# mantasu/face-crop-plus

Measured on AMD Instinct MI355X. Metric: faces/sec end-to-end (detect+align+crop), higher is better.
Workload: dtype f16x3; 1 GPU; RetinaFace detect + 5-pt align/crop, batch=32/GPU synthetic 1024x1024 RGB, strategy=largest, det_threshold=0.6, output 256x256, detector on 2 HIP streams x 16 images; global_batch=32, image_size=1024, parallelism=dp1

## Files before the change

face-crop-plus_amd/csrc/fcp_stem_pool.hip:

```cpp
#include "fcp_conv_common.h"

using namespace fcp_conv;

namespace {

typedef _Float16 f16x2 __attribute__((ext_vector_type(2)));

constexpr int PH = 5;
constexpr int SH = 2 * PH + 1;
constexpr int IH = 2 * SH + 5;
constexpr int SPITCH = 68;
constexpr int KSTEPS = 11;

struct StemGeo {
  static constexpr int PW = 16;
  static constexpr int SW = 2 * PW + 1;
  static constexpr int NSTEM = SH * SW;
  static constexpr int NTILES = (NSTEM + 31) / 32;
  static constexpr int IWB = (2 * SW + 5) * 3;
  static constexpr int IPITCH = 6 * SW + 18;
  static constexpr int IN_ELEMS = (IH + 1) * IPITCH;
  static constexpr int NT = 32 * PW;
  static constexpr int NGRP = NT / 128;
  static constexpr int TPR = NT / 28;
  static constexpr int NLOAD = (IWB + TPR - 1) / TPR;
  static constexpr int C1ROWS = (PH * PW + 31) / 32 * 32;
  static constexpr int C1_BYTES = C1ROWS * 2 * 128;
  static constexpr int WGS = 1;
  static_assert(TPR % 3 == 0 && IH * TPR <= NT && IPITCH % 2 == 0 && NTILES % NGRP == 0, "stem patch geometry");
};

struct StemParams {
  const uint8_t* img;
  const float* imgf;
  const uint32_t* wfrag;
  const float* bias;
  const float* wscale;
  float* out;
  int n, h, w, hs, ws, hp, wp, out_ld, out_fmt;
  int tiles_y, tiles_x, npatches;
  int mean[3];
  const char* w1;
  const float* ws1;
  const float* b1;
  float* t1;
  int t1_ld;
};

constexpr int CPITCH = 68;
__device__ __forceinline__ int swz1(int row) { return ((row >> 1) & 7) ^ ((row & 1) << 2); }

__device__ __forceinline__ void lds_barrier() {
  asm volatile("s_waitcnt lgkmcnt(0)" ::: "memory");
  __builtin_amdgcn_s_barrier();
  asm volatile("" ::: "memory");
}

template <bool HAS_C1, bool F32IN = false>
__global__ void __launch_bounds__(StemGeo::NT, StemGeo::WGS) stem_pool_kernel(const StemParams p) {
  static_assert(!(HAS_C1 && F32IN), "the fp32-input stem has no conv1 tail");
  using G = StemGeo;
  constexpr int PW = G::PW, SW = G::SW, NSTEM = G::NSTEM, NTILES = G::NTILES, IWB = G::IWB, IPITCH = G::IPITCH;
  constexpr int IN_ELEMS = G::IN_ELEMS, NT = G::NT, NGRP = G::NGRP, TPR = G::TPR, NLOAD = G::NLOAD, C1ROWS = G::C1ROWS;
  constexpr int KPG = NTILES / NGRP;
  extern __shared__ __attribute__((aligned(16))) float smem[];
  __shared__ __attribute__((aligned(16))) _Float16 inh[IN_ELEMS];
  __shared__ __attribute__((aligned(16))) _Float16 inl[F32IN ? IN_ELEMS : 8];
  float* stage = smem;
  char* c1in = reinterpret_cast<char*>(smem + NSTEM * SPITCH);

  const int tid = threadIdx.x;
  const int lane = tid & 63;
  const int wave = __builtin_amdgcn_readfirstlane(tid >> 6);
  const int half = lane >> 5;

  const int ct = wave & 1, grp = wave >> 1;
  f16x8 wh[KSTEPS], wl[KSTEPS];
#pragma unroll
  for (int q = 0; q < KSTEPS; ++q) {
    const u32x4_t* src = reinterpret_cast<const u32x4_t*>(p.wfrag) + ((ct * KSTEPS + q) * 2) * 64 + lane;
    wh[q] = __builtin_bit_cast(f16x8, src[0]);
    wl[q] = __builtin_bit_cast(f16x8, src[64]);
  }

  const int pc2 = 2 * (tid & 31), pcol = tid >> 5;
  const float ws2a = p.wscale[pc2], ws2b = p.wscale[pc2 + 1], bias2a = p.bias[pc2], bias2b = p.bias[pc2 + 1];
  float ws1a = 0.f, ws1b = 0.f, b1a = 0.f, b1b = 0.f;
  if constexpr (HAS_C1) { ws1a = p.ws1[pc2]; ws1b = p.ws1[pc2 + 1]; b1a = p.b1[pc2]; b1b = p.b1[pc2 + 1]; }
  const int c1rt = wave >> 1, c1ct = wave & 1;

  const int frow = tid / TPR, fc0 = tid - frow * TPR;
  const int fx0 = fc0 / 3, fch = fc0 - fx0 * 3;
  const int fmean = fch == 0 ? p.mean[0] : (fch == 1 ? p.mean[1] : p.mean[2]);
  _Float16* const fdst = inh + min(frow, IH - 1) * IPITCH + fc0;
  uint8_t pre[F32IN ? 1 : NLOAD];
  float pref[F32IN ? NLOAD : 1];
  unsigned pre_ok = 0u;
  auto fetch = [&](int patch) {
    const int pxi = patch % p.tiles_x;
    const int pyi = (patch / p.tiles_x) % p.tiles_y;
    const int ni = patch / (p.tiles_x * p.tiles_y);
    const int iy0 = 4 * pyi * PH - 5, ix0 = 4 * pxi * PW - 5;
    const int y = iy0 + frow;
    const bool rowok = (unsigned)y < (unsigned)p.h && frow < IH;
    const int yc = min(max(y, 0), p.h - 1);
    const uint8_t* base = p.img + ((long)ni * p.h + yc) * p.w * 3 + fch;
    const float* basef = p.imgf + ((long)ni * p.h + yc) * p.w * 4 + fch;
    pre_ok = 0u;
#pragma unroll
    for (int j = 0; j < NLOAD; ++j) {
      const int x = ix0 + fx0 + (TPR / 3) * j;
      pre_ok |= (rowok && (unsigned)x < (unsigned)p.w) ? (1u << j) : 0u;
      if constexpr (F32IN) pref[j] = basef[(unsigned)(min(max(x, 0), p.w - 1) * 4)];
      else pre[j] = base[(unsigned)(min(max(x, 0), p.w - 1) * 3)];
    }
  };
  _Float16* const fdstl = inl + (F32IN ? min(frow, IH - 1) * IPITCH + fc0 : 0);
  auto commit = [&]() {
    if (frow < IH) {
#pragma unroll
      for (int j = 0; j < NLOAD; ++j) {
        if (fc0 + TPR * j < IWB) {
          if constexpr (F32IN) {
            const float v = ((pre_ok >> j) & 1u) ? pref[j] : 0.f;
            const unsigned hu = __builtin_bit_cast(unsigned, __builtin_amdgcn_cvt_pkrtz(v, 0.f));
            const unsigned lu = __builtin_bit_cast(unsigned, __builtin_amdgcn_cvt_pkrtz(fcp_mix_diff<0>(v, hu), 0.f));
            fdst[TPR * j] = __builtin_bit_cast(_Float16, (unsigned short)(hu & 0xFFFFu));
            fdstl[TPR * j] = __builtin_bit_cast(_Float16, (unsigned short)(lu & 0xFFFFu));
          } else {
            fdst[TPR * j] = (_Float16)(float)(((pre_ok >> j) & 1u) ? (int)pre[j] - fmean : 0);
          }
        }
      }
    }
  };

  for (int i = tid; i < IN_ELEMS / 2; i += NT) {
    reinterpret_cast<uint32_t*>(inh)[i] = 0u;
    if constexpr (F32IN) reinterpret_cast<uint32_t*>(inl)[i] = 0u;
  }
  __syncthreads();

  int abase_t[KPG];
#pragma unroll
  for (int k = 0; k < KPG; ++k) {
    int pix = (grp + NGRP * k) * 32 + (lane & 31);
    pix = pix < NSTEM ? pix : NSTEM - 1;
    const int si = pix / SW, sj = pix - si * SW;
    abase_t[k] = (2 * si) * IPITCH + 6 * sj;
  }

  int patch = blockIdx.x;
  if (patch < p.npatches) fetch(patch);
  for (; patch < p.npatches; patch += gridDim.x) {
    commit();
    lds_barrier();
    const int next = patch + gridDim.x;
    if (next < p.npatches) fetch(next);

    const int pxi = patch % p.tiles_x;
    const int pyi = (patch / p.tiles_x) % p.tiles_y;
    const int ni = patch / (p.tiles_x * p.tiles_y);
    const int py0 = pyi * PH, px0 = pxi * PW;
    const int sy0 = 2 * py0 - 1, sx0 = 2 * px0 - 1;
    const bool interior = sy0 >= 0 && sy0 + SH <= p.hs && sx0 >= 0 && sx0 + SW <= p.ws;

#pragma unroll
    for (int k = 0; k < KPG; ++k) {
      const int t = grp + NGRP * k;
      const int abase = abase_t[k];
      f32x16 acc;
#pragma unroll
      for (int e = 0; e < 16; ++e) acc[e] = 0.f;
      auto afrag_of = [&](const _Float16* plane, int q) {
        const int ch = 2 * q + half;
        const int kh = ch / 3, part = ch - kh * 3;
        const uint32_t* wp = reinterpret_cast<const uint32_t*>(plane + abase + kh * IPITCH + 8 * part);
        const u32x4_t raw = {wp[0], wp[1], wp[2], wp[3]};
        return __builtin_bit_cast(f16x8, raw);
      };
      auto afrag = [&](int q) { return afrag_of(inh, q); };
      f16x8 a = afrag(0), al = a;
      if constexpr (F32IN) al = afrag_of(inl, 0);
#pragma unroll
      for (int q = 0; q < KSTEPS; ++q) {
        f16x8 an = a, aln = al;
        if (q + 1 < KSTEPS) {
          an = afrag(q + 1);
          if constexpr (F32IN) aln = afrag_of(inl, q + 1);
        }
        __builtin_amdgcn_sched_barrier(0);
        if constexpr (F32IN) {
          acc = __builtin_amdgcn_mfma_f32_32x32x16_f16(wh[q], al, acc, 0, 0, 0);
          acc = __builtin_amdgcn_mfma_f32_32x32x16_f16(wl[q], a, acc, 0, 0, 0);
          acc = __builtin_amdgcn_mfma_f32_32x32x16_f16(wh[q], a, acc, 0, 0, 0);
        } else {
          acc = __builtin_amdgcn_mfma_f32_32x32x16_f16(wl[q], a, acc, 0, 0, 0);
          acc = __builtin_amdgcn_mfma_f32_32x32x16_f16(wh[q], a, acc, 0, 0, 0);
        }
        a = an; al = aln;
      }
      {
        const int row = t * 32 + (lane & 31);
        bool in = true;
        if (!interior) {
          const int si = row / SW, sj = row - si * SW;
          in = (unsigned)(sy0 + si) < (unsigned)p.hs && (unsigned)(sx0 + sj) < (unsigned)p.ws;
        }
        if (row < NSTEM) {
          float* dst = stage + row * SPITCH + ct * 32 + 4 * half;
#pragma unroll
          for (int g = 0; g < 4; ++g)
            *reinterpret_cast<f32x4*>(dst + 8 * g) = in ? f32x4{acc[4 * g], acc[4 * g + 1], acc[4 * g + 2], acc[4 * g + 3]}
                                                        : f32x4{-INFINITY, -INFINITY, -INFINITY, -INFINITY};
        }
      }
    }
    lds_barrier();

    f16x8 c1w[8];
    if constexpr (HAS_C1) {
      if (c1rt < C1ROWS / 32) {
        const char* wrow = p.w1 + (size_t)(c1ct * 32 + (lane & 31)) * 256;
#pragma unroll
        for (int sl = 0; sl < 2; ++sl)
#pragma unroll
          for (int sh = 0; sh < 2; ++sh) {
            c1w[(sl * 2 + sh) * 2] = *reinterpret_cast<const f16x8*>(wrow + sl * 128 + (2 * sh + half) * 16);
            c1w[(sl * 2 + sh) * 2 + 1] = *reinterpret_cast<const f16x8*>(wrow + sl * 128 + (4 + 2 * sh + half) * 16);
          }
      }
    }
    {
      typedef float f32x2 __attribute__((ext_vector_type(2)));
      const float* sp = stage + (2 * pcol) * SPITCH + pc2;
      f32x2 rm[SH];
#pragma unroll
      for (int si = 0; si < SH; ++si) {
        const f32x2 a = *reinterpret_cast<const f32x2*>(sp + (si * SW) * SPITCH);
        const f32x2 b = *reinterpret_cast<const f32x2*>(sp + (si * SW + 1) * SPITCH);
        const f32x2 c = *reinterpret_cast<const f32x2*>(sp + (si * SW + 2) * SPITCH);
        rm[si][0] = fmaxf(fmaxf(a[0], b[0]), c[0]);
        rm[si][1] = fmaxf(fmaxf(a[1], b[1]), c[1]);
      }
      const int ox = px0 + pcol;
#pragma unroll
      for (int py = 0; py < PH; ++py) {
        const int oy = py0 + py;
        if (oy >= p.hp || ox >= p.wp) continue;
        float v0 = fmaxf(fmaxf(rm[2 * py][0], rm[2 * py + 1][0]), rm[2 * py + 2][0]) * ws2a + bias2a;
        float v1 = fmaxf(fmaxf(rm[2 * py][1], rm[2 * py + 1][1]), rm[2 * py + 2][1]) * ws2b + bias2b;
        v0 = v0 > 0.f ? v0 : 0.f;
        v1 = v1 > 0.f ? v1 : 0.f;
        const long pixel = ((long)ni * p.hp + oy) * p.wp + ox;
        if (p.out_fmt == 1) {
          unsigned hu, lu;
          split2(v0, v1, hu, lu);
          char* ob = reinterpret_cast<char*>(p.out) + pixel * p.out_ld * 4 + split_chan_off(pc2);
          *reinterpret_cast<unsigned*>(ob) = hu;
          *reinterpret_cast<unsigned*>(ob + 64) = lu;
          if constexpr (HAS_C1) {
            const int pp = py * PW + pcol;
            const int q = (pc2 & 31) >> 3, sw = swz1(pp);
            char* trow = c1in + pp * 256 + (pc2 >> 5) * 128 + (pc2 & 7) * 2;
            *reinterpret_cast<unsigned*>(trow + ((q ^ sw) << 4)) = hu;
            *reinterpret_cast<unsigned*>(trow + (((4 + q) ^ sw) << 4)) = lu;
          }
        } else {
          *reinterpret_cast<f32x2*>(p.out + pixel * p.out_ld + pc2) = f32x2{v0, v1};
        }
      }
    }
    if constexpr (HAS_C1) {
      lds_barrier();
      if (c1rt < C1ROWS / 32) {
        f32x16 acc;
#pragma unroll
        for (int e = 0; e < 16; ++e) acc[e] = 0.f;
        const int row = c1rt * 32 + (lane & 31), sw = swz1(row);
        const char* arow = c1in + row * 256;
#pragma unroll
        for (int sl = 0; sl < 2; ++sl)
#pragma unroll
          for (int sh = 0; sh < 2; ++sh) {
            const f16x8 bh = c1w[(sl * 2 + sh) * 2], bl = c1w[(sl * 2 + sh) * 2 + 1];
            const f16x8 ah = *reinterpret_cast<const f16x8*>(arow + sl * 128 + (((2 * sh + half) ^ sw) << 4));
            const f16x8 al = *reinterpret_cast<const f16x8*>(arow + sl * 128 + (((4 + 2 * sh + half) ^ sw) << 4));
            acc = __builtin_amdgcn_mfma_f32_32x32x16_f16(bh, al, acc, 0, 0, 0);
            acc = __builtin_amdgcn_mfma_f32_32x32x16_f16(bl, ah, acc, 0, 0, 0);
            acc = __builtin_amdgcn_mfma_f32_32x32x16_f16(bh, ah, acc, 0, 0, 0);
          }
        float* dst = stage + row * CPITCH + c1ct * 32 + 4 * half;
#pragma unroll
        for (int g = 0; g < 4; ++g)
          *reinterpret_cast<f32x4*>(dst + 8 * g) = f32x4{acc[4 * g], acc[4 * g + 1], acc[4 * g + 2], acc[4 * g + 3]};
      }
      lds_barrier();
      {
        typedef float f32x2 __attribute__((ext_vector_type(2)));
        const int ox = px0 + pcol;
        f32x2 cv[PH];
#pragma unroll
        for (int py = 0; py < PH; ++py) cv[py] = *reinterpret_cast<const f32x2*>(stage + (py * PW + pcol) * CPITCH + pc2);
#pragma unroll
        for (int py = 0; py < PH; ++py) {
          const int oy = py0 + py;
          if (oy >= p.hp || ox >= p.wp) continue;
          const float x0 = conv_value_relu(cv[py][0], ws1a, b1a), x1 = conv_value_relu(cv[py][1], ws1b, b1b);
          unsigned hu, lu;
          split2(x0, x1, hu, lu);
          const long pixel = ((long)ni * p.hp + oy) * p.wp + ox;
          char* ob = reinterpret_cast<char*>(p.t1) + pixel * p.t1_ld * 4 + split_chan_off(pc2);
          *reinterpret_cast<unsigned*>(ob) = hu;
          *reinterpret_cast<unsigned*>(ob + 64) = lu;
        }
      }
    }
    lds_barrier();
  }
}

}

extern "C" int fcp_stem7x7s2_relu_pool_conv1_u8(const uint8_t* images, int n, int h, int w, const int32_t* mean_rgb,
                                                const void* wfrag, const float* bias, const float* wscale, float* out,
                                                int out_ld, int out_fmt, const void* w1, const float* ws1, const float* b1,
                                                float* t1, int t1_ld, fcp_stream_t stream) {
  FCP_REQUIRE(images && wfrag && bias && wscale && out && mean_rgb, "stem: null pointer");
  const bool has_c1 = w1 != nullptr;
  if (has_c1) {
    FCP_REQUIRE(ws1 && b1 && t1, "stem + conv1: conv1 needs its scales, bias and output");
    FCP_REQUIRE(out_fmt == 1, "stem + conv1: the pooled map must be written in split32 (its bytes are conv1's operand)");
    FCP_REQUIRE(t1_ld >= 64 && t1_ld % 32 == 0 && ((uintptr_t)t1 & 127) == 0 && ((uintptr_t)w1 & 15) == 0,
                "stem + conv1: misaligned conv1 filter / output view");
  }
  FCP_REQUIRE(n > 0 && h >= 1 && w >= 1 && (long)h * w * 3 < (1L << 31), "stem: bad image size");
  FCP_REQUIRE((unsigned)out_fmt <= 1u, "stem: out_fmt must be 0 (fp32) or 1 (split32)");
  FCP_REQUIRE(out_ld >= 64 && out_ld % (out_fmt ? 32 : 4) == 0 && ((uintptr_t)out & (out_fmt ? 127 : 15)) == 0,
              "stem: misaligned output view");
  FCP_REQUIRE(((uintptr_t)wfrag & 15) == 0, "stem: filter fragments must be 16-byte aligned");
  for (int c = 0; c < 3; ++c) FCP_REQUIRE(mean_rgb[c] >= 0 && mean_rgb[c] <= 255, "stem: means must be integers in 0..255");
  StemParams p = {};
  p.img = images; p.wfrag = static_cast<const uint32_t*>(wfrag); p.bias = bias; p.wscale = wscale; p.out = out;
  p.n = n; p.h = h; p.w = w;
  p.hs = (h + 6 - 7) / 2 + 1; p.ws = (w + 6 - 7) / 2 + 1;
  p.hp = (p.hs + 2 - 3) / 2 + 1; p.wp = (p.ws + 2 - 3) / 2 + 1;
  p.out_ld = out_ld; p.out_fmt = out_fmt;
  p.tiles_y = fcp_cdiv(p.hp, PH); p.tiles_x = fcp_cdiv(p.wp, StemGeo::PW);
  const long np = (long)n * p.tiles_y * p.tiles_x;
  FCP_REQUIRE(np < (1L << 31) && (long)n * h * w * 3 < (1L << 40), "stem: batch too large");
  p.npatches = (int)np;
  for (int c = 0; c < 3; ++c) p.mean[c] = mean_rgb[c];
  p.w1 = static_cast<const char*>(w1); p.ws1 = ws1; p.b1 = b1; p.t1 = t1; p.t1_ld = t1_ld;
  using G = StemGeo;
  const size_t lds = (size_t)G::NSTEM * SPITCH * 4 + (has_c1 ? G::C1_BYTES : 0);
  const int cus = fcp_cu_count() * G::WGS;
  const int grid = (int)(np < cus ? np : cus);
  if (has_c1) {
    FCP_LDS_OPT_IN((&stem_pool_kernel<true>), lds);
    hipLaunchKernelGGL((stem_pool_kernel<true>), dim3(grid), dim3(G::NT), lds, (hipStream_t)stream, p);
  } else {
    FCP_LDS_OPT_IN((&stem_pool_kernel<false>), lds);
    hipLaunchKernelGGL((stem_pool_kernel<false>), dim3(grid), dim3(G::NT), lds, (hipStream_t)stream, p);
  }
  FCP_LAUNCH_OK();
  return 0;
}

extern "C" int fcp_stem7x7s2_relu_pool_f32(const float* x4, int n, int h, int w, const void* wfrag, const float* bias,
                                           const float* wscale, float* out, int out_ld, int out_fmt, fcp_stream_t stream) {
  FCP_REQUIRE(x4 && wfrag && bias && wscale && out, "stem(f32): null pointer");
  FCP_REQUIRE(n > 0 && h >= 1 && w >= 1 && (long)h * w * 4 < (1L << 31), "stem(f32): bad image size");
  FCP_REQUIRE((unsigned)out_fmt <= 1u, "stem(f32): out_fmt must be 0 (fp32) or 1 (split32)");
  FCP_REQUIRE(out_ld >= 64 && out_ld % (out_fmt ? 32 : 4) == 0 && ((uintptr_t)out & (out_fmt ? 127 : 15)) == 0,
              "stem(f32): misaligned output view");
  FCP_REQUIRE(((uintptr_t)wfrag & 15) == 0 && ((uintptr_t)x4 & 15) == 0, "stem(f32): input / filter fragments must be 16-byte aligned");
  using G = StemGeo;
  StemParams p = {};
  p.imgf = x4; p.wfrag = static_cast<const uint32_t*>(wfrag); p.bias = bias; p.wscale = wscale; p.out = out;
  p.n = n; p.h = h; p.w = w;
  p.hs = (h + 6 - 7) / 2 + 1; p.ws = (w + 6 - 7) / 2 + 1;
  p.hp = (p.hs + 2 - 3) / 2 + 1; p.wp = (p.ws + 2 - 3) / 2 + 1;
  p.out_ld = out_ld; p.out_fmt = out_fmt;
  p.tiles_y = fcp_cdiv(p.hp, PH); p.tiles_x = fcp_cdiv(p.wp, G::PW);
  const long np = (long)n * p.tiles_y * p.tiles_x;
  FCP_REQUIRE(np < (1L << 31) && (long)n * h * w * 4 < (1L << 40), "stem(f32): batch too large");
  p.npatches = (int)np;
  const size_t lds = (size_t)G::NSTEM * SPITCH * 4;
  const int cus = fcp_cu_count() * G::WGS;
  const int grid = (int)(np < cus ? np : cus);
  FCP_LDS_OPT_IN((&stem_pool_kernel<false, true>), lds);
  hipLaunchKernelGGL((stem_pool_kernel<false, true>), dim3(grid), dim3(G::NT), lds, (hipStream_t)stream, p);
  FCP_LAUNCH_OK();
  return 0;
}

extern "C" int fcp_stem7x7s2_relu_pool_u8(const uint8_t* images, int n, int h, int w, const int32_t* mean_rgb,
                                          const void* wfrag, const float* bias, const float* wscale, float* out,
                                          int out_ld, int out_fmt, fcp_stream_t stream) {
  return fcp_stem7x7s2_relu_pool_conv1_u8(images, n, h, w, mean_rgb, wfrag, bias, wscale, out, out_ld, out_fmt, nullptr, nullptr,
                                          nullptr, nullptr, 0, stream);
}
```

Baseline: 1454 faces/s.

## Coalesce stem-pool and conv1 output stores via LDS-staged 16-byte writes

In the fused stem+conv1 path, the pooled map is no longer written to global memory with scattered 4-byte stores per thread. Instead it is copied out of the LDS conv1 operand tile in 16-byte pieces with nontemporal stores after the barrier. The conv1 epilogue now has each thread handle 8 channels of one pixel for the first rows and pack them with pack_store8, and the last row keeps the old path with nontemporal stores. This aims to cut store-instruction count and improve coalescing, at the cost of more index arithmetic and a new 16-byte alignment requirement on ws1/b1.

```diff
diff --git a/face-crop-plus_amd/csrc/fcp_stem_pool.hip b/face-crop-plus_amd/csrc/fcp_stem_pool.hip
--- a/face-crop-plus_amd/csrc/fcp_stem_pool.hip
+++ b/face-crop-plus_amd/csrc/fcp_stem_pool.hip
@@ -256,15 +256,16 @@
         if (p.out_fmt == 1) {
           unsigned hu, lu;
           split2(v0, v1, hu, lu);
-          char* ob = reinterpret_cast<char*>(p.out) + pixel * p.out_ld * 4 + split_chan_off(pc2);
-          *reinterpret_cast<unsigned*>(ob) = hu;
-          *reinterpret_cast<unsigned*>(ob + 64) = lu;
           if constexpr (HAS_C1) {
             const int pp = py * PW + pcol;
             const int q = (pc2 & 31) >> 3, sw = swz1(pp);
             char* trow = c1in + pp * 256 + (pc2 >> 5) * 128 + (pc2 & 7) * 2;
             *reinterpret_cast<unsigned*>(trow + ((q ^ sw) << 4)) = hu;
             *reinterpret_cast<unsigned*>(trow + (((4 + q) ^ sw) << 4)) = lu;
+          } else {
+            char* ob = reinterpret_cast<char*>(p.out) + pixel * p.out_ld * 4 + split_chan_off(pc2);
+            *reinterpret_cast<unsigned*>(ob) = hu;
+            *reinterpret_cast<unsigned*>(ob + 64) = lu;
           }
         } else {
           *reinterpret_cast<f32x2*>(p.out + pixel * p.out_ld + pc2) = f32x2{v0, v1};
@@ -273,6 +274,26 @@
     }
     if constexpr (HAS_C1) {
       lds_barrier();
+      int tid1 = tid;
+      asm volatile("" : "+v"(tid1));
+      {
+        constexpr int NPIECE = PH * PW * 16;
+        char* const ob = reinterpret_cast<char*>(p.out);
+#pragma unroll
+        for (int k = 0; k < (NPIECE + NT - 1) / NT; ++k) {
+          const int item = tid1 + NT * k;
+          const int pp = item >> 4, piece = item & 15;
+          const int oy = py0 + pp / PW, ox = px0 + pp % PW;
+          if (item < NPIECE && oy < p.hp && ox < p.wp) {
+            const u32x4_t v = *reinterpret_cast<const u32x4_t*>(c1in + pp * 256 + (piece & 8) * 16 + (((piece & 7) ^ swz1(pp)) << 4));
+            const long pixel = ((long)ni * p.hp + oy) * p.wp + ox;
+            __builtin_nontemporal_store(v, reinterpret_cast<u32x4_t*>(ob + pixel * p.out_ld * 4 + piece * 16));
+          }
+        }
+      }
+      const int c8 = 8 * (tid1 & 7);
+      const f32x4 ws1lo = *reinterpret_cast<const f32x4*>(p.ws1 + c8), ws1hi = *reinterpret_cast<const f32x4*>(p.ws1 + c8 + 4);
+      const f32x4 b1lo = *reinterpret_cast<const f32x4*>(p.b1 + c8), b1hi = *reinterpret_cast<const f32x4*>(p.b1 + c8 + 4);
       if (c1rt < C1ROWS / 32) {
         f32x16 acc;
 #pragma unroll
@@ -297,22 +318,33 @@
       }
       lds_barrier();
       {
+        const int pp = tid1 >> 3;
+        const int oy = py0 + pp / PW, ox = px0 + pp % PW;
+        if (oy < p.hp && ox < p.wp) {
+          const f32x4 a = *reinterpret_cast<const f32x4*>(stage + pp * CPITCH + c8);
+          const f32x4 b = *reinterpret_cast<const f32x4*>(stage + pp * CPITCH + c8 + 4);
+          float v[8];
+#pragma unroll
+          for (int e = 0; e < 4; ++e) {
+            v[e] = conv_value_relu(a[e], ws1lo[e], b1lo[e]);
+            v[4 + e] = conv_value_relu(b[e], ws1hi[e], b1hi[e]);
+          }
+          const long pixel = ((long)ni * p.hp + oy) * p.wp + ox;
+          pack_store8(p.t1, pixel, p.t1_ld, c8, 1, 1, v);
+        }
+      }
+      {
         typedef float f32x2 __attribute__((ext_vector_type(2)));
-        const int ox = px0 + pcol;
-        f32x2 cv[PH];
-#pragma unroll
-        for (int py = 0; py < PH; ++py) cv[py] = *reinterpret_cast<const f32x2*>(stage + (py * PW + pcol) * CPITCH + pc2);
-#pragma unroll
-        for (int py = 0; py < PH; ++py) {
-          const int oy = py0 + py;
-          if (oy >= p.hp || ox >= p.wp) continue;
-          const float x0 = conv_value_relu(cv[py][0], ws1a, b1a), x1 = conv_value_relu(cv[py][1], ws1b, b1b);
+        const int oy = py0 + PH - 1, ox = px0 + pcol;
+        if (oy < p.hp && ox < p.wp) {
+          const f32x2 cv = *reinterpret_cast<const f32x2*>(stage + ((PH - 1) * PW + pcol) * CPITCH + pc2);
+          const float x0 = conv_value_relu(cv[0], ws1a, b1a), x1 = conv_value_relu(cv[1], ws1b, b1b);
           unsigned hu, lu;
           split2(x0, x1, hu, lu);
           const long pixel = ((long)ni * p.hp + oy) * p.wp + ox;
           char* ob = reinterpret_cast<char*>(p.t1) + pixel * p.t1_ld * 4 + split_chan_off(pc2);
-          *reinterpret_cast<unsigned*>(ob) = hu;
-          *reinterpret_cast<unsigned*>(ob + 64) = lu;
+          __builtin_nontemporal_store(hu, reinterpret_cast<unsigned*>(ob));
+          __builtin_nontemporal_store(lu, reinterpret_cast<unsigned*>(ob + 64));
         }
       }
     }
@@ -333,6 +365,7 @@
     FCP_REQUIRE(out_fmt == 1, "stem + conv1: the pooled map must be written in split32 (its bytes are conv1's operand)");
     FCP_REQUIRE(t1_ld >= 64 && t1_ld % 32 == 0 && ((uintptr_t)t1 & 127) == 0 && ((uintptr_t)w1 & 15) == 0,
                 "stem + conv1: misaligned conv1 filter / output view");
+    FCP_REQUIRE((((uintptr_t)ws1 | (uintptr_t)b1) & 15) == 0, "stem + conv1: conv1's scales and bias must be 16-byte aligned");
   }
   FCP_REQUIRE(n > 0 && h >= 1 && w >= 1 && (long)h * w * 3 < (1L << 31), "stem: bad image size");
   FCP_REQUIRE((unsigned)out_fmt <= 1u, "stem: out_fmt must be 0 (fp32) or 1 (split32)");
```

Result: no change. 1455 faces/s (median of 6 runs) (+0.1%).

## Warp-specialize stem kernel into conv producer and pool/conv1 consumer waves

Applied to the files above, without the earlier changes.

Splits the 512-thread stem block into four MFMA conv waves and four service waves. The conv waves fill double-buffered input and stage tiles, and the service waves do max-pool, output writes and the conv1 tail on the previous patch, so the two phases overlap. The patch height shrinks to fit the doubled LDS buffers. Conv1 now runs per wave on private LDS with wave-local ordering instead of block barriers. This trades smaller tiles, more halo overhead and half the MFMA waves for overlap across stages.

```diff
diff --git a/face-crop-plus_amd/csrc/fcp_stem_pool.hip b/face-crop-plus_amd/csrc/fcp_stem_pool.hip
--- a/face-crop-plus_amd/csrc/fcp_stem_pool.hip
+++ b/face-crop-plus_amd/csrc/fcp_stem_pool.hip
@@ -5,8 +5,9 @@
 namespace {
 
 typedef _Float16 f16x2 __attribute__((ext_vector_type(2)));
-
-constexpr int PH = 5;
+typedef float f32x2 __attribute__((ext_vector_type(2)));
+
+constexpr int PH = 3;
 constexpr int SH = 2 * PH + 1;
 constexpr int IH = 2 * SH + 5;
 constexpr int SPITCH = 68;
@@ -20,14 +21,22 @@
   static constexpr int IWB = (2 * SW + 5) * 3;
   static constexpr int IPITCH = 6 * SW + 18;
   static constexpr int IN_ELEMS = (IH + 1) * IPITCH;
-  static constexpr int NT = 32 * PW;
-  static constexpr int NGRP = NT / 128;
-  static constexpr int TPR = NT / 28;
+  static constexpr int NT = 512;
+  static constexpr int NROLE = NT / 2;
+  static constexpr int NGRP = NROLE / 128;
+  static constexpr int KPG = NTILES / NGRP;
+  static constexpr int TPR = NROLE / IH / 3 * 3;
   static constexpr int NLOAD = (IWB + TPR - 1) / TPR;
-  static constexpr int C1ROWS = (PH * PW + 31) / 32 * 32;
-  static constexpr int C1_BYTES = C1ROWS * 2 * 128;
+  static constexpr int WCOLS = PW / 4;
+  static constexpr int C1_WAVE_BYTES = 16 * 256;
+  static constexpr int STAGE_ELEMS = NSTEM * SPITCH;
   static constexpr int WGS = 1;
-  static_assert(TPR % 3 == 0 && IH * TPR <= NT && IPITCH % 2 == 0 && NTILES % NGRP == 0, "stem patch geometry");
+  static_assert(TPR % 3 == 0 && IH * TPR <= NROLE && IPITCH % 2 == 0 && NTILES % (2 * NGRP) == 0, "stem patch geometry");
+  static_assert(PH * WCOLS <= 16 && PH * WCOLS * SPITCH * 4 <= C1_WAVE_BYTES && WCOLS == 4, "conv1 tail geometry");
+  static_assert(STAGE_ELEMS % 4 == 0 && IN_ELEMS % 8 == 0, "LDS regions stay 16-byte aligned");
+  static constexpr size_t lds_bytes(bool has_c1, bool f32in) {
+    return (size_t)2 * STAGE_ELEMS * 4 + (size_t)(f32in ? 4 : 2) * IN_ELEMS * 2 + (has_c1 ? 4 * C1_WAVE_BYTES : 0);
+  }
 };
 
 struct StemParams {
@@ -55,269 +64,343 @@
   __builtin_amdgcn_s_barrier();
   asm volatile("" ::: "memory");
 }
+__device__ __forceinline__ void lds_wave_order() { asm volatile("s_waitcnt lgkmcnt(0)" ::: "memory"); }
 
 template <bool HAS_C1, bool F32IN = false>
 __global__ void __launch_bounds__(StemGeo::NT, StemGeo::WGS) stem_pool_kernel(const StemParams p) {
   static_assert(!(HAS_C1 && F32IN), "the fp32-input stem has no conv1 tail");
   using G = StemGeo;
-  constexpr int PW = G::PW, SW = G::SW, NSTEM = G::NSTEM, NTILES = G::NTILES, IWB = G::IWB, IPITCH = G::IPITCH;
-  constexpr int IN_ELEMS = G::IN_ELEMS, NT = G::NT, NGRP = G::NGRP, TPR = G::TPR, NLOAD = G::NLOAD, C1ROWS = G::C1ROWS;
-  constexpr int KPG = NTILES / NGRP;
+  constexpr int PW = G::PW, SW = G::SW, NSTEM = G::NSTEM, IWB = G::IWB, IPITCH = G::IPITCH;
+  constexpr int IN_ELEMS = G::IN_ELEMS, NT = G::NT, NGRP = G::NGRP, TPR = G::TPR, NLOAD = G::NLOAD, KPG = G::KPG;
+  constexpr int NPLANES = F32IN ? 2 : 1;
   extern __shared__ __attribute__((aligned(16))) float smem[];
-  __shared__ __attribute__((aligned(16))) _Float16 inh[IN_ELEMS];
-  __shared__ __attribute__((aligned(16))) _Float16 inl[F32IN ? IN_ELEMS : 8];
-  float* stage = smem;
-  char* c1in = reinterpret_cast<char*>(smem + NSTEM * SPITCH);
+  float* const stage0 = smem;
+  _Float16* const inh0 = reinterpret_cast<_Float16*>(smem + 2 * G::STAGE_ELEMS);
+  _Float16* const inl0 = inh0 + 2 * IN_ELEMS;
+  char* const c1lds = reinterpret_cast<char*>(inh0 + 2 * NPLANES * IN_ELEMS);
 
   const int tid = threadIdx.x;
   const int lane = tid & 63;
   const int wave = __builtin_amdgcn_readfirstlane(tid >> 6);
   const int half = lane >> 5;
-
-  const int ct = wave & 1, grp = wave >> 1;
-  f16x8 wh[KSTEPS], wl[KSTEPS];
-#pragma unroll
-  for (int q = 0; q < KSTEPS; ++q) {
-    const u32x4_t* src = reinterpret_cast<const u32x4_t*>(p.wfrag) + ((ct * KSTEPS + q) * 2) * 64 + lane;
-    wh[q] = __builtin_bit_cast(f16x8, src[0]);
-    wl[q] = __builtin_bit_cast(f16x8, src[64]);
+  const bool service = wave >= 4;
+
+  for (int i = tid; i < NPLANES * IN_ELEMS; i += NT) reinterpret_cast<uint32_t*>(inh0)[i] = 0u;
+  __syncthreads();
+
+  const int cnt = (p.npatches - (int)blockIdx.x + (int)gridDim.x - 1) / (int)gridDim.x;
+  const int tiles_xy = p.tiles_x * p.tiles_y;
+
+  if (!service) {
+    const int ct = wave & 1, grp = wave >> 1;
+    f16x8 wh[KSTEPS], wl[KSTEPS];
+#pragma unroll
+    for (int q = 0; q < KSTEPS; ++q) {
+      const u32x4_t* src = reinterpret_cast<const u32x4_t*>(p.wfrag) + ((ct * KSTEPS + q) * 2) * 64 + lane;
+      wh[q] = __builtin_bit_cast(f16x8, src[0]);
+      wl[q] = __builtin_bit_cast(f16x8, src[64]);
+    }
+    int abase_t[KPG];
+#pragma unroll
+    for (int k = 0; k < KPG; ++k) {
+      int pix = (grp + NGRP * k) * 32 + (lane & 31);
+      pix = pix < NSTEM ? pix : NSTEM - 1;
+      const int si = pix / SW, sj = pix - si * SW;
+      abase_t[k] = (2 * si) * IPITCH + 6 * sj;
+    }
+
+    const int frow = tid / TPR, fc0 = tid - frow * TPR;
+    const int fx0 = fc0 / 3, fch = fc0 - fx0 * 3;
+    const int fmean = fch == 0 ? p.mean[0] : (fch == 1 ? p.mean[1] : p.mean[2]);
+    const int foff = min(frow, IH - 1) * IPITCH + fc0;
+    uint8_t pre[F32IN ? 1 : NLOAD];
+    float pref[F32IN ? NLOAD : 1];
+    unsigned pre_ok = 0u;
+    auto fetch = [&](int patch) {
+      const int pxi = patch % p.tiles_x;
+      const int pyi = (patch / p.tiles_x) % p.tiles_y;
+      const int ni = patch / tiles_xy;
+      const int iy0 = 4 * pyi * PH - 5, ix0 = 4 * pxi * PW - 5;
+      const int y = iy0 + frow;
+      const bool rowok = (unsigned)y < (unsigned)p.h && frow < IH;
+      const int yc = min(max(y, 0), p.h - 1);
+      const uint8_t* base = p.img + ((long)ni * p.h + yc) * p.w * 3 + fch;
+      const float* basef = p.imgf + ((long)ni * p.h + yc) * p.w * 4 + fch;
+      unsigned ok = 0u;
+#pragma unroll
+      for (int j = 0; j < NLOAD; ++j) {
+        const int x = ix0 + fx0 + (TPR / 3) * j;
+        ok |= (rowok && (unsigned)x < (unsigned)p.w) ? (1u << j) : 0u;
+        if constexpr (F32IN) pref[j] = basef[(unsigned)(min(max(x, 0), p.w - 1) * 4)];
+        else pre[j] = base[(unsigned)(min(max(x, 0), p.w - 1) * 3)];
+      }
+      pre_ok = ok;
+    };
+    auto commit = [&](int s) {
+      _Float16* const fdst = inh0 + s * IN_ELEMS + foff;
+      _Float16* const fdstl = inl0 + s * IN_ELEMS + foff;
+      const unsigned ok = pre_ok;
+      if (frow < IH) {
+#pragma unroll
+        for (int j = 0; j < NLOAD; ++j) {
+          if (fc0 + TPR * j < IWB) {
+            if constexpr (F32IN) {
+              const float v = ((ok >> j) & 1u) ? pref[j] : 0.f;
+              const unsigned hu = __builtin_bit_cast(unsigned, __builtin_amdgcn_cvt_pkrtz(v, 0.f));
+              const unsigned lu = __builtin_bit_cast(unsigned, __builtin_amdgcn_cvt_pkrtz(fcp_mix_diff<0>(v, hu), 0.f));
+              fdst[TPR * j] = __builtin_bit_cast(_Float16, (unsigned short)(hu & 0xFFFFu));
+              fdstl[TPR * j] = __builtin_bit_cast(_Float16, (unsigned short)(lu & 0xFFFFu));
+            } else {
+              fdst[TPR * j] = (_Float16)(float)(((ok >> j) & 1u) ? (int)pre[j] - fmean : 0);
+            }
+          }
+        }
+      }
+    };
+
+    fetch(blockIdx.x);
+    commit(0);
+    if (cnt > 1) fetch(blockIdx.x + gridDim.x);
+    lds_barrier();
+
+    for (int i = 0; i <= cnt; ++i) {
+      if (i < cnt) {
+        const int patch = blockIdx.x + i * gridDim.x;
+        const int pxi = patch % p.tiles_x;
+        const int pyi = (patch / p.tiles_x) % p.tiles_y;
+        const int sy0 = 2 * pyi * PH - 1, sx0 = 2 * pxi * PW - 1;
+        const bool interior = sy0 >= 0 && sy0 + SH <= p.hs && sx0 >= 0 && sx0 + SW <= p.ws;
+        const _Float16* inh = inh0 + (i & 1) * IN_ELEMS;
+        const _Float16* inl = inl0 + (i & 1) * IN_ELEMS;
+        float* stage = stage0 + (i & 1) * G::STAGE_ELEMS;
+
+#pragma unroll
+        for (int kp = 0; kp < KPG; kp += 2) {
+          f32x16 acc[2];
+#pragma unroll
+          for (int u = 0; u < 2; ++u)
+#pragma unroll
+            for (int e = 0; e < 16; ++e) acc[u][e] = 0.f;
+          auto afrag_of = [&](const _Float16* plane, int u, int q) {
+            const int ch = 2 * q + half;
+            const int kh = ch / 3, part = ch - kh * 3;
+            const uint32_t* wp = reinterpret_cast<const uint32_t*>(plane + abase_t[kp + u] + kh * IPITCH + 8 * part);
+            const u32x4_t raw = {wp[0], wp[1], wp[2], wp[3]};
+            return __builtin_bit_cast(f16x8, raw);
+          };
+          f16x8 a[2], al[2];
+#pragma unroll
+          for (int u = 0; u < 2; ++u) {
+            a[u] = afrag_of(inh, u, 0);
+            al[u] = a[u];
+            if constexpr (F32IN) al[u] = afrag_of(inl, u, 0);
+          }
+#pragma unroll
+          for (int q = 0; q < KSTEPS; ++q) {
+            f16x8 an[2] = {a[0], a[1]}, aln[2] = {al[0], al[1]};
+            if (q + 1 < KSTEPS) {
+#pragma unroll
+              for (int u = 0; u < 2; ++u) {
+                an[u] = afrag_of(inh, u, q + 1);
+                if constexpr (F32IN) aln[u] = afrag_of(inl, u, q + 1);
+              }
+            }
+            __builtin_amdgcn_sched_barrier(0);
+            if constexpr (F32IN) {
+              acc[0] = __builtin_amdgcn_mfma_f32_32x32x16_f16(wh[q], al[0], acc[0], 0, 0, 0);
+              acc[1] = __builtin_amdgcn_mfma_f32_32x32x16_f16(wh[q], al[1], acc[1], 0, 0, 0);
+              acc[0] = __builtin_amdgcn_mfma_f32_32x32x16_f16(wl[q], a[0], acc[0], 0, 0, 0);
+              acc[1] = __builtin_amdgcn_mfma_f32_32x32x16_f16(wl[q], a[1], acc[1], 0, 0, 0);
+              acc[0] = __builtin_amdgcn_mfma_f32_32x32x16_f16(wh[q], a[0], acc[0], 0, 0, 0);
+              acc[1] = __builtin_amdgcn_mfma_f32_32x32x16_f16(wh[q], a[1], acc[1], 0, 0, 0);
+            } else {
+              acc[0] = __builtin_amdgcn_mfma_f32_32x32x16_f16(wl[q], a[0], acc[0], 0, 0, 0);
+              acc[1] = __builtin_amdgcn_mfma_f32_32x32x16_f16(wl[q], a[1], acc[1], 0, 0, 0);
+              acc[0] = __builtin_amdgcn_mfma_f32_32x32x16_f16(wh[q], a[0], acc[0], 0, 0, 0);
+              acc[1] = __builtin_amdgcn_mfma_f32_32x32x16_f16(wh[q], a[1], acc[1], 0, 0, 0);
+            }
+#pragma unroll
+            for (int u = 0; u < 2; ++u) { a[u] = an[u]; al[u] = aln[u]; }
+          }
+#pragma unroll
+          for (int u = 0; u < 2; ++u) {
+            const int row = (grp + NGRP * (kp + u)) * 32 + (lane & 31);
+            bool in = true;
+            if (!interior) {
+              const int si = row / SW, sj = row - si * SW;
+              in = (unsigned)(sy0 + si) < (unsigned)p.hs && (unsigned)(sx0 + sj) < (unsigned)p.ws;
+            }
+            if (row < NSTEM) {
+              float* dst = stage + row * SPITCH + ct * 32 + 4 * half;
+#pragma unroll
+              for (int g = 0; g < 4; ++g)
+                *reinterpret_cast<f32x4*>(dst + 8 * g) = in ? f32x4{acc[u][4 * g], acc[u][4 * g + 1], acc[u][4 * g + 2], acc[u][4 * g + 3]}
+                                                            : f32x4{-INFINITY, -INFINITY, -INFINITY, -INFINITY};
+            }
+          }
+        }
+        if (i + 1 < cnt) commit((i + 1) & 1);
+        if (i + 2 < cnt) fetch(blockIdx.x + (i + 2) * gridDim.x);
+      }
+      lds_barrier();
+    }
+    return;
   }
 
-  const int pc2 = 2 * (tid & 31), pcol = tid >> 5;
+  const int sw4 = wave - 4;
+  const int pc2 = 2 * (lane & 31), pcl = 2 * half, pcol = G::WCOLS * sw4 + pcl;
   const float ws2a = p.wscale[pc2], ws2b = p.wscale[pc2 + 1], bias2a = p.bias[pc2], bias2b = p.bias[pc2 + 1];
   float ws1a = 0.f, ws1b = 0.f, b1a = 0.f, b1b = 0.f;
   if constexpr (HAS_C1) { ws1a = p.ws1[pc2]; ws1b = p.ws1[pc2 + 1]; b1a = p.b1[pc2]; b1b = p.b1[pc2 + 1]; }
-  const int c1rt = wave >> 1, c1ct = wave & 1;
-
-  const int frow = tid / TPR, fc0 = tid - frow * TPR;
-  const int fx0 = fc0 / 3, fch = fc0 - fx0 * 3;
-  const int fmean = fch == 0 ? p.mean[0] : (fch == 1 ? p.mean[1] : p.mean[2]);
-  _Float16* const fdst = inh + min(frow, IH - 1) * IPITCH + fc0;
-  uint8_t pre[F32IN ? 1 : NLOAD];
-  float pref[F32IN ? NLOAD : 1];
-  unsigned pre_ok = 0u;
-  auto fetch = [&](int patch) {
-    const int pxi = patch % p.tiles_x;
-    const int pyi = (patch / p.tiles_x) % p.tiles_y;
-    const int ni = patch / (p.tiles_x * p.tiles_y);
-    const int iy0 = 4 * pyi * PH - 5, ix0 = 4 * pxi * PW - 5;
-    const int y = iy0 + frow;
-    const bool rowok = (unsigned)y < (unsigned)p.h && frow < IH;
-    const int yc = min(max(y, 0), p.h - 1);
-    const uint8_t* base = p.img + ((long)ni * p.h + yc) * p.w * 3 + fch;
-    const float* basef = p.imgf + ((long)ni * p.h + yc) * p.w * 4 + fch;
-    pre_ok = 0u;
-#pragma unroll
-    for (int j = 0; j < NLOAD; ++j) {
-      const int x = ix0 + fx0 + (TPR / 3) * j;
-      pre_ok |= (rowok && (unsigned)x < (unsigned)p.w) ? (1u << j) : 0u;
-      if constexpr (F32IN) pref[j] = basef[(unsigned)(min(max(x, 0), p.w - 1) * 4)];
-      else pre[j] = base[(unsigned)(min(max(x, 0), p.w - 1) * 3)];
+  char* const c1in = c1lds + (HAS_C1 ? sw4 * G::C1_WAVE_BYTES : 0);
+  f16x8 c1w[2][8];
+  if constexpr (HAS_C1) {
+#pragma unroll
+    for (int c = 0; c < 2; ++c) {
+      const char* wrow = p.w1 + (size_t)(c * 32 + (lane & 31)) * 256;
+#pragma unroll
+      for (int sl = 0; sl < 2; ++sl)
+#pragma unroll
+        for (int sh = 0; sh < 2; ++sh) {
+          c1w[c][(sl * 2 + sh) * 2] = *reinterpret_cast<const f16x8*>(wrow + sl * 128 + (2 * sh + half) * 16);
+          c1w[c][(sl * 2 + sh) * 2 + 1] = *reinterpret_cast<const f16x8*>(wrow + sl * 128 + (4 + 2 * sh + half) * 16);
+        }
     }
-  };
-  _Float16* const fdstl = inl + (F32IN ? min(frow, IH - 1) * IPITCH + fc0 : 0);
-  auto commit = [&]() {
-    if (frow < IH) {
-#pragma unroll
-      for (int j = 0; j < NLOAD; ++j) {
-        if (fc0 + TPR * j < IWB) {
-          if constexpr (F32IN) {
-            const float v = ((pre_ok >> j) & 1u) ? pref[j] : 0.f;
-            const unsigned hu = __builtin_bit_cast(unsigned, __builtin_amdgcn_cvt_pkrtz(v, 0.f));
-            const unsigned lu = __builtin_bit_cast(unsigned, __builtin_amdgcn_cvt_pkrtz(fcp_mix_diff<0>(v, hu), 0.f));
-            fdst[TPR * j] = __builtin_bit_cast(_Float16, (unsigned short)(hu & 0xFFFFu));
-            fdstl[TPR * j] = __builtin_bit_cast(_Float16, (unsigned short)(lu & 0xFFFFu));
-          } else {
-            fdst[TPR * j] = (_Float16)(float)(((pre_ok >> j) & 1u) ? (int)pre[j] - fmean : 0);
+  }
+
+  lds_barrier();
+
+  for (int i = 0; i <= cnt; ++i) {
+    if (i >= 1) {
+      const int patch = blockIdx.x + (i - 1) * gridDim.x;
+      const int pxi = patch % p.tiles_x;
+      const int pyi = (patch / p.tiles_x) % p.tiles_y;
+      const int ni = patch / tiles_xy;
+      const int py0 = pyi * PH, px0 = pxi * PW;
+      const float* stage = stage0 + ((i - 1) & 1) * G::STAGE_ELEMS;
+
+      {
+        const float* sp = stage + (2 * pcol) * SPITCH + pc2;
+        f32x2 rm[2][SH];
+#pragma unroll
+        for (int si = 0; si < SH; ++si) {
+          f32x2 r[5];
+#pragma unroll
+          for (int j = 0; j < 5; ++j) r[j] = *reinterpret_cast<const f32x2*>(sp + (si * SW + j) * SPITCH);
+#pragma unroll
+          for (int c = 0; c < 2; ++c) {
+            rm[c][si][0] = fmaxf(fmaxf(r[2 * c][0], r[2 * c + 1][0]), r[2 * c + 2][0]);
+            rm[c][si][1] = fmaxf(fmaxf(r[2 * c][1], r[2 * c + 1][1]), r[2 * c + 2][1]);
+          }
+        }
+#pragma unroll
+        for (int py = 0; py < PH; ++py) {
+#pragma unroll
+          for (int c = 0; c < 2; ++c) {
+            const int oy = py0 + py, ox = px0 + pcol + c;
+            if (oy >= p.hp || ox >= p.wp) continue;
+            float v0 = fmaxf(fmaxf(rm[c][2 * py][0], rm[c][2 * py + 1][0]), rm[c][2 * py + 2][0]) * ws2a + bias2a;
+            float v1 = fmaxf(fmaxf(rm[c][2 * py][1], rm[c][2 * py + 1][1]), rm[c][2 * py + 2][1]) * ws2b + bias2b;
+            v0 = v0 > 0.f ? v0 : 0.f;
+            v1 = v1 > 0.f ? v1 : 0.f;
+            const long pixel = ((long)ni * p.hp + oy) * p.wp + ox;
+            if (p.out_fmt == 1) {
+              unsigned hu, lu;
+              split2(v0, v1, hu, lu);
+              char* ob = reinterpret_cast<char*>(p.out) + pixel * p.out_ld * 4 + split_chan_off(pc2);
+              *reinterpret_cast<unsigned*>(ob) = hu;
+              *reinterpret_cast<unsigned*>(ob + 64) = lu;
+              if constexpr (HAS_C1) {
+                const int pp = py * G::WCOLS + pcl + c;
+                const int q = (pc2 & 31) >> 3, sw = swz1(pp);
+                char* trow = c1in + pp * 256 + (pc2 >> 5) * 128 + (pc2 & 7) * 2;
+                *reinterpret_cast<unsigned*>(trow + ((q ^ sw) << 4)) = hu;
+                *reinterpret_cast<unsigned*>(trow + (((4 + q) ^ sw) << 4)) = lu;
+              }
+            } else {
+              *reinterpret_cast<f32x2*>(p.out + pixel * p.out_ld + pc2) = f32x2{v0, v1};
+            }
           }
         }
       }
-    }
-  };
-
-  for (int i = tid; i < IN_ELEMS / 2; i += NT) {
-    reinterpret_cast<uint32_t*>(inh)[i] = 0u;
-    if constexpr (F32IN) reinterpret_cast<uint32_t*>(inl)[i] = 0u;
-  }
-  __syncthreads();
-
-  int abase_t[KPG];
-#pragma unroll
-  for (int k = 0; k < KPG; ++k) {
-    int pix = (grp + NGRP * k) * 32 + (lane & 31);
-    pix = pix < NSTEM ? pix : NSTEM - 1;
-    const int si = pix / SW, sj = pix - si * SW;
-    abase_t[k] = (2 * si) * IPITCH + 6 * sj;
-  }
-
-  int patch = blockIdx.x;
-  if (patch < p.npatches) fetch(patch);
-  for (; patch < p.npatches; patch += gridDim.x) {
-    commit();
-    lds_barrier();
-    const int next = patch + gridDim.x;
-    if (next < p.npatches) fetch(next);
-
-    const int pxi = patch % p.tiles_x;
-    const int pyi = (patch / p.tiles_x) % p.tiles_y;
-    const int ni = patch / (p.tiles_x * p.tiles_y);
-    const int py0 = pyi * PH, px0 = pxi * PW;
-    const int sy0 = 2 * py0 - 1, sx0 = 2 * px0 - 1;
-    const bool interior = sy0 >= 0 && sy0 + SH <= p.hs && sx0 >= 0 && sx0 + SW <= p.ws;
-
-#pragma unroll
-    for (int k = 0; k < KPG; ++k) {
-      const int t = grp + NGRP * k;
-      const int abase = abase_t[k];
-      f32x16 acc;
-#pragma unroll
-      for (int e = 0; e < 16; ++e) acc[e] = 0.f;
-      auto afrag_of = [&](const _Float16* plane, int q) {
-        const int ch = 2 * q + half;
-        const int kh = ch / 3, part = ch - kh * 3;
-        const uint32_t* wp = reinterpret_cast<const uint32_t*>(plane + abase + kh * IPITCH + 8 * part);
-        const u32x4_t raw = {wp[0], wp[1], wp[2], wp[3]};
-        return __builtin_bit_cast(f16x8, raw);
-      };
-      auto afrag = [&](int q) { return afrag_of(inh, q); };
-      f16x8 a = afrag(0), al = a;
-      if constexpr (F32IN) al = afrag_of(inl, 0);
-#pragma unroll
-      for (int q = 0; q < KSTEPS; ++q) {
-        f16x8 an = a, aln = al;
-        if (q + 1 < KSTEPS) {
-          an = afrag(q + 1);
-          if constexpr (F32IN) aln = afrag_of(inl, q + 1);
-        }
-        __builtin_amdgcn_sched_barrier(0);
-        if constexpr (F32IN) {
-          acc = __builtin_amdgcn_mfma_f32_32x32x16_f16(wh[q], al, acc, 0, 0, 0);
-          acc = __builtin_amdgcn_mfma_f32_32x32x16_f16(wl[q], a, acc, 0, 0, 0);
-          acc = __builtin_amdgcn_mfma_f32_32x32x16_f16(wh[q], a, acc, 0, 0, 0);
-        } else {
-          acc = __builtin_amdgcn_mfma_f32_32x32x16_f16(wl[q], a, acc, 0, 0, 0);
-          acc = __builtin_amdgcn_mfma_f32_32x32x16_f16(wh[q], a, acc, 0, 0, 0);
-        }
-        a = an; al = aln;
-      }
-      {
-        const int row = t * 32 + (lane & 31);
-        bool in = true;
-        if (!interior) {
-          const int si = row / SW, sj = row - si * SW;
-          in = (unsigned)(sy0 + si) < (unsigned)p.hs && (unsigned)(sx0 + sj) < (unsigned)p.ws;
-        }
-        if (row < NSTEM) {
-          float* dst = stage + row * SPITCH + ct * 32 + 4 * half;
-#pragma unroll
-          for (int g = 0; g < 4; ++g)
-            *reinterpret_cast<f32x4*>(dst + 8 * g) = in ? f32x4{acc[4 * g], acc[4 * g + 1], acc[4 * g + 2], acc[4 * g + 3]}
-                                                        : f32x4{-INFINITY, -INFINITY, -INFINITY, -INFINITY};
-        }
-      }
-    }
-    lds_barrier();
-
-    f16x8 c1w[8];
-    if constexpr (HAS_C1) {
-      if (c1rt < C1ROWS / 32) {
-        const char* wrow = p.w1 + (size_t)(c1ct * 32 + (lane & 31)) * 256;
+      if constexpr (HAS_C1) {
+        lds_wave_order();
+        const int row = lane & 31, orow = row & 15, sw = swz1(orow);
+        const char* arow = c1in + orow * 256;
+        f16x8 ah[4], al[4];
 #pragma unroll
         for (int sl = 0; sl < 2; ++sl)
 #pragma unroll
           for (int sh = 0; sh < 2; ++sh) {
-            c1w[(sl * 2 + sh) * 2] = *reinterpret_cast<const f16x8*>(wrow + sl * 128 + (2 * sh + half) * 16);
-            c1w[(sl * 2 + sh) * 2 + 1] = *reinterpret_cast<const f16x8*>(wrow + sl * 128 + (4 + 2 * sh + half) * 16);
-          }
-      }
-    }
-    {
-      typedef float f32x2 __attribute__((ext_vector_type(2)));
-      const float* sp = stage + (2 * pcol) * SPITCH + pc2;
-      f32x2 rm[SH];
-#pragma unroll
-      for (int si = 0; si < SH; ++si) {
-        const f32x2 a = *reinterpret_cast<const f32x2*>(sp + (si * SW) * SPITCH);
-        const f32x2 b = *reinterpret_cast<const f32x2*>(sp + (si * SW + 1) * SPITCH);
-        const f32x2 c = *reinterpret_cast<const f32x2*>(sp + (si * SW + 2) * SPITCH);
-        rm[si][0] = fmaxf(fmaxf(a[0], b[0]), c[0]);
-        rm[si][1] = fmaxf(fmaxf(a[1], b[1]), c[1]);
-      }
-      const int ox = px0 + pcol;
-#pragma unroll
-      for (int py = 0; py < PH; ++py) {
-        const int oy = py0 + py;
-        if (oy >= p.hp || ox >= p.wp) continue;
-        float v0 = fmaxf(fmaxf(rm[2 * py][0], rm[2 * py + 1][0]), rm[2 * py + 2][0]) * ws2a + bias2a;
-        float v1 = fmaxf(fmaxf(rm[2 * py][1], rm[2 * py + 1][1]), rm[2 * py + 2][1]) * ws2b + bias2b;
-        v0 = v0 > 0.f ? v0 : 0.f;
-        v1 = v1 > 0.f ? v1 : 0.f;
-        const long pixel = ((long)ni * p.hp + oy) * p.wp + ox;
-        if (p.out_fmt == 1) {
-          unsigned hu, lu;
-          split2(v0, v1, hu, lu);
-          char* ob = reinterpret_cast<char*>(p.out) + pixel * p.out_ld * 4 + split_chan_off(pc2);
-          *reinterpret_cast<unsigned*>(ob) = hu;
-          *reinterpret_cast<unsigned*>(ob + 64) = lu;
-          if constexpr (HAS_C1) {
-            const int pp = py * PW + pcol;
-            const int q = (pc2 & 31) >> 3, sw = swz1(pp);
-            char* trow = c1in + pp * 256 + (pc2 >> 5) * 128 + (pc2 & 7) * 2;
-            *reinterpret_cast<unsigned*>(trow + ((q ^ sw) << 4)) = hu;
-            *reinterpret_cast<unsigned*>(trow + (((4 + q) ^ sw) << 4)) = lu;
-          }
-        } else {
-          *reinterpret_cast<f32x2*>(p.out + pixel * p.out_ld + pc2) = f32x2{v0, v1};
-        }
-      }
-    }
-    if constexpr (HAS_C1) {
-      lds_barrier();
-      if (c1rt < C1ROWS / 32) {
-        f32x16 acc;
-#pragma unroll
-        for (int e = 0; e < 16; ++e) acc[e] = 0.f;
-        const int row = c1rt * 32 + (lane & 31), sw = swz1(row);
-        const char* arow = c1in + row * 256;
-#pragma unroll
-        for (int sl = 0; sl < 2; ++sl)
-#pragma unroll
-          for (int sh = 0; sh < 2; ++sh) {
-            const f16x8 bh = c1w[(sl * 2 + sh) * 2], bl = c1w[(sl * 2 + sh) * 2 + 1];
-            const f16x8 ah = *reinterpret_cast<const f16x8*>(arow + sl * 128 + (((2 * sh + half) ^ sw) << 4));
-            const f16x8 al = *reinterpret_cast<const f16x8*>(arow + sl * 128 + (((4 + 2 * sh + half) ^ sw) << 4));
-            acc = __builtin_amdgcn_mfma_f32_32x32x16_f16(bh, al, acc, 0, 0, 0);
-            acc = __builtin_amdgcn_mfma_f32_32x32x16_f16(bl, ah, acc, 0, 0, 0);
-            acc = __builtin_amdgcn_mfma_f32_32x32x16_f16(bh, ah, acc, 0, 0, 0);
-          }
-        float* dst = stage + row * CPITCH + c1ct * 32 + 4 * half;
-#pragma unroll
-        for (int g = 0; g < 4; ++g)
-          *reinterpret_cast<f32x4*>(dst + 8 * g) = f32x4{acc[4 * g], acc[4 * g + 1], acc[4 * g + 2], acc[4 * g + 3]};
-      }
-      lds_barrier();
-      {
-        typedef float f32x2 __attribute__((ext_vector_type(2)));
-        const int ox = px0 + pcol;
-        f32x2 cv[PH];
-#pragma unroll
-        for (int py = 0; py < PH; ++py) cv[py] = *reinterpret_cast<const f32x2*>(stage + (py * PW + pcol) * CPITCH + pc2);
+            ah[sl * 2 + sh] = *reinterpret_cast<const f16x8*>(arow + sl * 128 + (((2 * sh + half) ^ sw) << 4));
+            al[sl * 2 + sh] = *reinterpret_cast<const f16x8*>(arow + sl * 128 + (((4 + 2 * sh + half) ^ sw) << 4));
+          }
+        lds_wave_order();
+        float* const cst = reinterpret_cast<float*>(c1in);
+#pragma unroll
+        for (int c = 0; c < 2; ++c) {
+          f32x16 acc;
+#pragma unroll
+          for (int e = 0; e < 16; ++e) acc[e] = 0.f;
+#pragma unroll
+          for (int s = 0; s < 4; ++s) {
+            const f16x8 bh = c1w[c][s * 2], bl = c1w[c][s * 2 + 1];
+            acc = __builtin_amdgcn_mfma_f32_32x32x16_f16(bh, al[s], acc, 0, 0, 0);
+            acc = __builtin_amdgcn_mfma_f32_32x32x16_f16(bl, ah[s], acc, 0, 0, 0);
+            acc = __builtin_amdgcn_mfma_f32_32x32x16_f16(bh, ah[s], acc, 0, 0, 0);
+          }
+          if (row < PH * G::WCOLS) {
+            float* dst = cst + row * CPITCH + c * 32 + 4 * half;
+#pragma unroll
+            for (int g = 0; g < 4; ++g)
+              *reinterpret_cast<f32x4*>(dst + 8 * g) = f32x4{acc[4 * g], acc[4 * g + 1], acc[4 * g + 2], acc[4 * g + 3]};
+          }
+        }
+        lds_wave_order();
+        f32x2 cv[PH][2];
+#pragma unroll
+        for (int py = 0; py < PH; ++py)
+#pragma unroll
+          for (int c = 0; c < 2; ++c) cv[py][c] = *reinterpret_cast<const f32x2*>(cst + (py * G::WCOLS + pcl + c) * CPITCH + pc2);
+        lds_wave_order();
 #pragma unroll
         for (int py = 0; py < PH; ++py) {
-          const int oy = py0 + py;
-          if (oy >= p.hp || ox >= p.wp) continue;
-          const float x0 = conv_value_relu(cv[py][0], ws1a, b1a), x1 = conv_value_relu(cv[py][1], ws1b, b1b);
-          unsigned hu, lu;
-          split2(x0, x1, hu, lu);
-          const long pixel = ((long)ni * p.hp + oy) * p.wp + ox;
-          char* ob = reinterpret_cast<char*>(p.t1) + pixel * p.t1_ld * 4 + split_chan_off(pc2);
-          *reinterpret_cast<unsigned*>(ob) = hu;
-          *reinterpret_cast<unsigned*>(ob + 64) = lu;
+#pragma unroll
+          for (int c = 0; c < 2; ++c) {
+            const int oy = py0 + py, ox = px0 + pcol + c;
+            if (oy >= p.hp || ox >= p.wp) continue;
+            const float x0 = conv_value_relu(cv[py][c][0], ws1a, b1a), x1 = conv_value_relu(cv[py][c][1], ws1b, b1b);
+            unsigned hu, lu;
+            split2(x0, x1, hu, lu);
+            const long pixel = ((long)ni * p.hp + oy) * p.wp + ox;
+            char* ob = reinterpret_cast<char*>(p.t1) + pixel * p.t1_ld * 4 + split_chan_off(pc2);
+            *reinterpret_cast<unsigned*>(ob) = hu;
+            *reinterpret_cast<unsigned*>(ob + 64) = lu;
+          }
         }
       }
     }
     lds_barrier();
   }
+}
+
+template <bool HAS_C1, bool F32IN>
+int stem_launch(StemParams& p, fcp_stream_t stream) {
+  using G = StemGeo;
+  p.hs = (p.h + 6 - 7) / 2 + 1; p.ws = (p.w + 6 - 7) / 2 + 1;
+  p.hp = (p.hs + 2 - 3) / 2 + 1; p.wp = (p.ws + 2 - 3) / 2 + 1;
+  p.tiles_y = fcp_cdiv(p.hp, PH); p.tiles_x = fcp_cdiv(p.wp, G::PW);
+  const long np = (long)p.n * p.tiles_y * p.tiles_x;
+  FCP_REQUIRE(np < (1L << 31) && (long)p.n * p.h * p.w * (F32IN ? 4 : 3) < (1L << 40), "stem: batch too large");
+  p.npatches = (int)np;
+  constexpr size_t lds = G::lds_bytes(HAS_C1, F32IN);
+  static_assert(lds <= 160 * 1024, "stem: LDS budget");
+  const int cus = fcp_cu_count() * G::WGS;
+  const int grid = (int)(np < cus ? np : cus);
+  FCP_LDS_OPT_IN((&stem_pool_kernel<HAS_C1, F32IN>), lds);
+  hipLaunchKernelGGL((stem_pool_kernel<HAS_C1, F32IN>), dim3(grid), dim3(G::NT), lds, (hipStream_t)stream, p);
+  FCP_LAUNCH_OK();
+  return 0;
 }
 
 }
@@ -343,28 +426,10 @@
   StemParams p = {};
   p.img = images; p.wfrag = static_cast<const uint32_t*>(wfrag); p.bias = bias; p.wscale = wscale; p.out = out;
   p.n = n; p.h = h; p.w = w;
-  p.hs = (h + 6 - 7) / 2 + 1; p.ws = (w + 6 - 7) / 2 + 1;
-  p.hp = (p.hs + 2 - 3) / 2 + 1; p.wp = (p.ws + 2 - 3) / 2 + 1;
   p.out_ld = out_ld; p.out_fmt = out_fmt;
-  p.tiles_y = fcp_cdiv(p.hp, PH); p.tiles_x = fcp_cdiv(p.wp, StemGeo::PW);
-  const long np = (long)n * p.tiles_y * p.tiles_x;
-  FCP_REQUIRE(np < (1L << 31) && (long)n * h * w * 3 < (1L << 40), "stem: batch too large");
-  p.npatches = (int)np;
   for (int c = 0; c < 3; ++c) p.mean[c] = mean_rgb[c];
   p.w1 = static_cast<const char*>(w1); p.ws1 = ws1; p.b1 = b1; p.t1 = t1; p.t1_ld = t1_ld;
-  using G = StemGeo;
-  const size_t lds = (size_t)G::NSTEM * SPITCH * 4 + (has_c1 ? G::C1_BYTES : 0);
-  const int cus = fcp_cu_count() * G::WGS;
-  const int grid = (int)(np < cus ? np : cus);
-  if (has_c1) {
-    FCP_LDS_OPT_IN((&stem_pool_kernel<true>), lds);
-    hipLaunchKernelGGL((stem_pool_kernel<true>), dim3(grid), dim3(G::NT), lds, (hipStream_t)stream, p);
-  } else {
-    FCP_LDS_OPT_IN((&stem_pool_kernel<false>), lds);
-    hipLaunchKernelGGL((stem_pool_kernel<false>), dim3(grid), dim3(G::NT), lds, (hipStream_t)stream, p);
-  }
-  FCP_LAUNCH_OK();
-  return 0;
+  return has_c1 ? stem_launch<true, false>(p, stream) : stem_launch<false, false>(p, stream);
 }
 
 extern "C" int fcp_stem7x7s2_relu_pool_f32(const float* x4, int n, int h, int w, const void* wfrag, const float* bias,
@@ -375,24 +440,11 @@
   FCP_REQUIRE(out_ld >= 64 && out_ld % (out_fmt ? 32 : 4) == 0 && ((uintptr_t)out & (out_fmt ? 127 : 15)) == 0,
               "stem(f32): misaligned output view");
   FCP_REQUIRE(((uintptr_t)wfrag & 15) == 0 && ((uintptr_t)x4 & 15) == 0, "stem(f32): input / filter fragments must be 16-byte aligned");
-  using G = StemGeo;
   StemParams p = {};
   p.imgf = x4; p.wfrag = static_cast<const uint32_t*>(wfrag); p.bias = bias; p.wscale = wscale; p.out = out;
   p.n = n; p.h = h; p.w = w;
-  p.hs = (h + 6 - 7) / 2 + 1; p.ws = (w + 6 - 7) / 2 + 1;
-  p.hp = (p.hs + 2 - 3) / 2 + 1; p.wp = (p.ws + 2 - 3) / 2 + 1;
   p.out_ld = out_ld; p.out_fmt = out_fmt;
-  p.tiles_y = fcp_cdiv(p.hp, PH); p.tiles_x = fcp_cdiv(p.wp, G::PW);
-  const long np = (long)n * p.tiles_y * p.tiles_x;
-  FCP_REQUIRE(np < (1L << 31) && (long)n * h * w * 4 < (1L << 40), "stem(f32): batch too large");
-  p.npatches = (int)np;
-  const size_t lds = (size_t)G::NSTEM * SPITCH * 4;
-  const int cus = fcp_cu_count() * G::WGS;
-  const int grid = (int)(np < cus ? np : cus);
-  FCP_LDS_OPT_IN((&stem_pool_kernel<false, true>), lds);
-  hipLaunchKernelGGL((stem_pool_kernel<false, true>), dim3(grid), dim3(G::NT), lds, (hipStream_t)stream, p);
-  FCP_LAUNCH_OK();
-  return 0;
+  return stem_launch<false, true>(p, stream);
 }
 
 extern "C" int fcp_stem7x7s2_relu_pool_u8(const uint8_t* images, int n, int h, int w, const int32_t* mean_rgb,
```

Result: no change. 1454 faces/s before, 1457 faces/s after (median of 6 runs) (+0.3%).
